# European-XFEL/xFrame

Hardware: AMD Instinct MI355X
Metric: MTIP iterations/sec, 128 q-shells x L_max=32 (higher is better)
Workload: dtype f64 (complex128); 1 GPU; BASELINE config 4: 128 shells x L_max=32, grid 128x64x128, 8 restarts per GPU on 3 streams, tutorial schedule (HIO/SW/ER, ft_stab on), fused step; restarts_per_gpu=8, restarts_total=8, streams_per_gpu=3, engines_take_turns=True, parallelism=restart-sharded x1, step_mode=fused

## Files before the change

### xframe_amd/csrc/k_hankel.hip

```cpp
#include "mtip_internal.h"
#include <vector>

void launch_hankel_mfma(mtip_ctx* c, const double2* in, double2* out, int inverse);

void launch_hankel(mtip_ctx* c, const double2* in, double2* out, int inverse) {
    ProfScope ps(c, "hankel");
    launch_hankel_mfma(c, in, out, inverse);
}

__global__ void __launch_bounds__(256) k_coeff_diff(const double2* __restrict__ a, const double2* __restrict__ b,
                                                    double2* __restrict__ out, int N, int nlm, long long total) {
    const long long idx = (long long)blockIdx.x * blockDim.x + threadIdx.x;
    if (idx >= total) return;
    const int q = (int)((idx / nlm) % N);
    double2 v = a[idx];
    if (q > 0) v = csub(v, b[idx]);
    out[idx] = v;
}

void launch_coeff_diff(mtip_ctx* c, const double2* a, const double2* b, double2* out) {
    const long long total = (long long)c->B * c->N * c->nlm;
    hipLaunchKernelGGL(k_coeff_diff, dim3((unsigned)div_up(total, 256)), dim3(256), 0, c->stream, a, b, out, c->N,
                       c->nlm, total);
}

#define HT_CT_MAX 5
#define HT_KC 16
#define HT_ROWS 128
#define HT_WS (HT_ROWS + 16)
#define HT_THREADS 512
#define HT_NW (HT_KC * HT_ROWS / HT_THREADS)

struct HankelTile32 { int l, cflat0; };

template <int HT_CT, bool SUB>
__global__ void __launch_bounds__(HT_THREADS) k_hankel_tile(const double* __restrict__ in, double* __restrict__ out,
                                                            const double* __restrict__ W,
                                                            const HankelTile32* __restrict__ tiles, int N, int Np, int L,
                                                            int B, int poffs, double scale, int sign,
                                                            const double* __restrict__ in_sub, const uint8_t* __restrict__ sub_mask) {
    constexpr int HT_COLS = 16 * HT_CT;
    constexpr int HT_XS = HT_COLS + 16;
    constexpr int HT_NX = (HT_KC * HT_COLS + HT_THREADS - 1) / HT_THREADS;
    __shared__ double Ws[2][HT_KC][HT_WS];
    __shared__ double Xs[2][HT_KC][HT_XS];
    __shared__ double Ss[SUB ? 2 : 1][SUB ? HT_KC : 1][HT_XS];
    const int tid = threadIdx.x;
    const int wave = tid >> 6, lane = tid & 63;
    const HankelTile32 tinfo = tiles[blockIdx.x];
    const int l = tinfo.l;
    const int k_base = blockIdx.y * HT_ROWS;
    const int ncl = 4 * l + 2;
    const int nlm2 = 2 * (L + 1) * (L + 1);
    const double* Wl = W + (size_t)l * Np * N;
    const int wrow = tid >> 5, wcol = (tid & 31) * 4;
    int xrow[HT_NX], xc[HT_NX];
    size_t xoff[HT_NX];
    bool xok[HT_NX], xsub[HT_NX];
#pragma unroll
    for (int j = 0; j < HT_NX; ++j) {
        const int e = tid + j * HT_THREADS;
        xrow[j] = e / HT_COLS;
        xc[j] = e - xrow[j] * HT_COLS;
        const int cflat = tinfo.cflat0 + xc[j];
        xok[j] = xrow[j] < HT_KC && cflat < B * ncl;
        const int b = xok[j] ? cflat / ncl : 0;
        const int within = xok[j] ? cflat - b * ncl : 0;
        xoff[j] = (size_t)b * N * nlm2 + 2 * (size_t)l * l + within;
        xsub[j] = SUB && (sub_mask == nullptr || sub_mask[b] != 0);
    }
    double rw0[HT_NW], rx0[HT_NX], rw1[HT_NW], rx1[HT_NX];
    double rs0[SUB ? HT_NX : 1], rs1[SUB ? HT_NX : 1];
    auto request = [&](int p0, double (&rw)[HT_NW], double (&rx)[HT_NX], double (&rs)[SUB ? HT_NX : 1]) {
        const int p = p0 + wrow;
        const bool p_ok = p < Np;
        const double* wr = Wl + (size_t)(p_ok ? p : 0) * N + k_base + wcol;
#pragma unroll
        for (int j = 0; j < HT_NW; ++j) rw[j] = (p_ok && k_base + wcol + j < N) ? wr[j] : 0.0;
#pragma unroll
        for (int j = 0; j < HT_NX; ++j) {
            const bool ok = xok[j] && p0 + xrow[j] < Np;
            const size_t o = xoff[j] + (size_t)(p0 + xrow[j] + poffs) * nlm2;
            rx[j] = ok ? in[o] : 0.0;
            if (SUB) {
                rs[j] = (ok && xsub[j]) ? in_sub[o] : 0.0;
                rx[j] -= rs[j];
            }
        }
    };
    auto deposit = [&](int buf, const double (&rw)[HT_NW], const double (&rx)[HT_NX], const double (&rs)[SUB ? HT_NX : 1]) {
#pragma unroll
        for (int j = 0; j < HT_NW; ++j) Ws[buf][wrow][wcol + j] = rw[j];
#pragma unroll
        for (int j = 0; j < HT_NX; ++j)
            if (xrow[j] < HT_KC) {
                Xs[buf][xrow[j]][xc[j]] = rx[j];
                if (SUB) Ss[buf][xrow[j]][xc[j]] = rs[j];
            }
    };
    const int li = lane & 15, kk = lane >> 4;
    v4f64 acc[HT_CT];
#pragma unroll
    for (int t = 0; t < HT_CT; ++t) acc[t] = v4f64{0.0, 0.0, 0.0, 0.0};
    auto multiply = [&](int buf) {
#pragma unroll
        for (int s = 0; s < HT_KC / 4; ++s) {
            const double af = Ws[buf][4 * s + kk][wave * 16 + li];
#pragma unroll
            for (int t = 0; t < HT_CT; ++t) {
                const double bf = Xs[buf][4 * s + kk][16 * t + li];
                acc[t] = __builtin_amdgcn_mfma_f64_16x16x4f64(af, bf, acc[t], 0, 0, 0);
            }
            if (SUB && wave == 0 && k_base == 0) {
                const double a0 = li == 0 ? af : 0.0;
#pragma unroll
                for (int t = 0; t < HT_CT; ++t) {
                    const double sf = Ss[buf][4 * s + kk][16 * t + li];
                    acc[t] = __builtin_amdgcn_mfma_f64_16x16x4f64(a0, sf, acc[t], 0, 0, 0);
                }
            }
        }
    };
    const int n_chunks = (Np + HT_KC - 1) / HT_KC;
    request(0, rw0, rx0, rs0);
    deposit(0, rw0, rx0, rs0);
    if (n_chunks > 1) request(HT_KC, rw1, rx1, rs1);
    if (n_chunks > 2) request(2 * HT_KC, rw0, rx0, rs0);
    __syncthreads();
    for (int i = 0; i < n_chunks; i += 2) {
        multiply(0);
        if (i + 1 < n_chunks) deposit(1, rw1, rx1, rs1);
        __syncthreads();
        if (i + 3 < n_chunks) request((i + 3) * HT_KC, rw1, rx1, rs1);
        if (i + 1 >= n_chunks) break;
        multiply(1);
        if (i + 2 < n_chunks) deposit(0, rw0, rx0, rs0);
        __syncthreads();
        if (i + 4 < n_chunks) request((i + 4) * HT_KC, rw0, rx0, rs0);
    }
    int r = l & 3;
    if (sign < 0) r = (4 - r) & 3;
    const bool is_im = (li & 1) != 0;
#pragma unroll
    for (int t = 0; t < HT_CT; ++t) {
        const int cflat = tinfo.cflat0 + 16 * t + li;
        const bool col_ok = cflat < B * ncl;
        const int b = col_ok ? cflat / ncl : 0;
        const int within = col_ok ? cflat - b * ncl : 0;
        const size_t col_off = (size_t)b * N * nlm2 + 2 * (size_t)l * l + within;
#pragma unroll
        for (int j = 0; j < 4; ++j) {
            double v = acc[t][j] * scale;
            const double partner = __shfl_xor(v, 1, 64);
            double o;
            if (r == 0) o = v;
            else if (r == 2) o = -v;
            else if (r == 1) o = is_im ? partner : -partner;
            else o = is_im ? -partner : partner;
            const int k = k_base + wave * 16 + kk + 4 * j;
            if (col_ok && k < N) out[col_off + (size_t)k * nlm2] = o;
        }
    }
}

bool hankel_has_difference(const mtip_ctx* c) { return c->d_htiles32 != nullptr; }

int hankel_row_blocks(const mtip_ctx* c) { return div_up(c->N, HT_ROWS); }

void launch_hankel_mfma_sub(mtip_ctx* c, const double2* in, const double2* in_sub, double2* out, int inverse, const uint8_t* sub_mask) {
    const dim3 grid((unsigned)c->n_htiles32, (unsigned)hankel_row_blocks(c));
#define HT_LAUNCH(CT, SUBF)                                                                                                  \
    hipLaunchKernelGGL((k_hankel_tile<CT, SUBF>), grid, dim3(HT_THREADS), 0, c->stream, reinterpret_cast<const double*>(in), \
                       reinterpret_cast<double*>(out), (const double*)c->d_W, (const HankelTile32*)c->d_htiles32, c->N,      \
                       c->Np, c->L, c->B, c->cfg.hankel_trapz ? 1 : 0, inverse ? c->inv_scale : c->fwd_scale,                \
                       inverse ? +1 : -1, reinterpret_cast<const double*>(in_sub), sub_mask)
    if (in_sub != nullptr) {
        switch (c->htile_ct) {
            case 1: HT_LAUNCH(1, true); break;
            case 2: HT_LAUNCH(2, true); break;
            case 3: HT_LAUNCH(3, true); break;
            default: HT_LAUNCH(5, true); break;
        }
    } else {
        switch (c->htile_ct) {
            case 1: HT_LAUNCH(1, false); break;
            case 2: HT_LAUNCH(2, false); break;
            case 3: HT_LAUNCH(3, false); break;
            default: HT_LAUNCH(5, false); break;
        }
    }
#undef HT_LAUNCH
}

void launch_hankel_mfma(mtip_ctx* c, const double2* in, double2* out, int inverse) {
    launch_hankel_mfma_sub(c, in, nullptr, out, inverse);
}

int build_hankel_tiles(mtip_ctx* c) {
    std::vector<HankelTile32> t32;
    const int cts[4] = {5, 3, 2, 1};
    for (int ci = 0; ci < 4; ++ci) {
        t32.clear();
        c->htile_ct = cts[ci];
        for (int l = c->L; l >= 0; --l) {
            const int ncols = c->B * (4 * l + 2);
            for (int c0 = 0; c0 < ncols; c0 += 16 * cts[ci]) t32.push_back(HankelTile32{l, c0});
        }
        if (c->htile_force > 0 ? cts[ci] == c->htile_force : (int)t32.size() * hankel_row_blocks(c) * 5 >= c->n_cu * 4) break;
    }
    {
        const int X = 8;
        std::vector<std::vector<HankelTile32>> q(X);
        size_t i0 = 0;
        while (i0 < t32.size()) {
            size_t i1 = i0;
            while (i1 < t32.size() && t32[i1].l == t32[i0].l) ++i1;
            int best = 0;
            for (int x = 1; x < X; ++x)
                if (q[x].size() < q[best].size()) best = x;
            q[best].insert(q[best].end(), t32.begin() + i0, t32.begin() + i1);
            i0 = i1;
        }
        std::vector<size_t> head(X, 0);
        std::vector<HankelTile32> order;
        while (order.size() < t32.size())
            for (int x = 0; x < X && order.size() < t32.size(); ++x) {
                if (head[x] < q[x].size()) { order.push_back(q[x][head[x]++]); continue; }
                int longest = 0;
                for (int y = 1; y < X; ++y)
                    if (q[y].size() - head[y] > q[longest].size() - head[longest]) longest = y;
                order.push_back(q[longest].back());
                q[longest].pop_back();
            }
        t32.swap(order);
    }
    c->n_htiles32 = (int)t32.size();
    if (c->d_htiles32.alloc(t32.size()) != hipSuccess) return MTIP_ENOMEM;
    (void)mtip_copy(c, c->d_htiles32, t32.data(), t32.size() * sizeof(HankelTile32), hipMemcpyHostToDevice);
    return MTIP_OK;
}
```

### xframe_amd/csrc/mtip_api.hip

```cpp
#include "mtip_internal.h"
#include <algorithm>
#include <cmath>
#include <cstdlib>
#include <cstring>

static thread_local std::string g_create_error;

#define CTX_CHECK(c)                       \
    do {                                   \
        if ((c) == nullptr) return MTIP_EINVAL; \
    } while (0)
#define FAIL(c, code, msg)      \
    do {                        \
        (c)->err = (msg);       \
        return (code);          \
    } while (0)

static int post_launch(mtip_ctx* c, const char* what) {
    hipError_t e = hipGetLastError();
    if (e != hipSuccess) {
        c->err = std::string(what) + ": " + hipGetErrorString(e);
        return MTIP_EHIP;
    }
    return MTIP_OK;
}

template <typename T>
static int dev_alloc(mtip_ctx* c, DevBuf<T>* p, size_t n) {
    const hipError_t e = p->alloc(n);
    if (e != hipSuccess) {
        c->err = std::string("hipMalloc: ") + hipGetErrorString(e);
        return MTIP_ENOMEM;
    }
    return MTIP_OK;
}

static ProjSwitches read_proj_switches() {
    ProjSwitches s;
    if (const char* e = std::getenv("MTIP_PROJ_FUSE")) s.fuse = std::atoi(e) != 0;
    if (const char* e = std::getenv("MTIP_JAC_RESIDENT")) s.jac_resident = std::atoi(e) != 0;
    if (const char* e = std::getenv("MTIP_JAC_TG")) s.jac_tg = std::atoi(e) == 8 ? 8 : 16;
    if (const char* e = std::getenv("MTIP_PROJ_REAL")) s.real = std::atoi(e) != 0;
    if (const char* e = std::getenv("MTIP_POLAR_ABS_TOL")) s.polar_abs_tol = std::atof(e);
    if (const char* e = std::getenv("MTIP_RP_CORR")) s.rp_corr = std::atoi(e) != 0;
    if (const char* e = std::getenv("MTIP_RP_EARLY")) s.rp_early = std::min(std::max(std::atof(e), 1e-3), 0.2);
    if (const char* e = std::getenv("MTIP_RP_CORR2_MAX")) s.rp_corr2_max = std::min(std::max(std::atof(e), 1e-6), 5e-4);
    return s;
}

extern "C" {

int mtip_device_count(void) {
    int n = 0;
    if (hipGetDeviceCount(&n) != hipSuccess) return 0;
    return n;
}

const char* mtip_last_error(const mtip_ctx* ctx) { return ctx ? ctx->err.c_str() : g_create_error.c_str(); }

void mtip_destroy(mtip_ctx* c) {
    if (!c) return;
    (void)hipSetDevice(c->device);
    if (c->stream) (void)hipStreamSynchronize(c->stream);
    for (hipEvent_t e : c->prof_events) (void)hipEventDestroy(e);
    if (c->ev0) (void)hipEventDestroy(c->ev0);
    if (c->ev1) (void)hipEventDestroy(c->ev1);
    if (c->turn_ev) (void)hipEventDestroy(c->turn_ev);
    if (c->stream) (void)hipStreamDestroy(c->stream);
    delete c;
}

static int require_loop_band_limit(mtip_ctx* c, const char* what) {
    if (c->L > MTIP_LOOP_L_MAX && !(c->cfg.reserved & MTIP_CFG_LOOP_BIG_L))
        FAIL(c, MTIP_ESTATE, std::string(what) + ": the phasing loop and the projection are built for max_order <= 63; this context has L = " +
                                 std::to_string(c->L) + " and runs the transforms only (DESIGN section 6)");
    return MTIP_OK;
}

static bool is_pow2(int v) { return v > 0 && (v & (v - 1)) == 0; }

mtip_ctx* mtip_create(const mtip_cfg* cfg, int device) {
    if (!cfg) {
        g_create_error = "cfg is NULL";
        return nullptr;
    }
    const int ndev = mtip_device_count();
    if (ndev <= 0) {
        g_create_error = "no HIP device visible (libmtip_hip needs an MI355X; there is no CPU fallback)";
        return nullptr;
    }
    if (device < 0 || device >= ndev) {
        g_create_error = "device index out of range";
        return nullptr;
    }
    if (cfg->n_radial < 2 || cfg->l_max < 0 || cfg->l_max > 128 || cfg->n_batch < 1 || !is_pow2(cfg->n_phi) ||
        cfg->n_phi < 4 || cfg->n_phi > 512 || cfg->n_phi <= 2 * cfg->l_max || cfg->n_theta <= cfg->l_max) {
        g_create_error = "invalid cfg: need Nq>=2, 0<=L<=128 (the transforms; the phasing loop and the projection: L<=63), n_batch>=1, n_phi a power of two in [4,512] and > 2L, n_theta > L";
        return nullptr;
    }
    if (cfg->reserved & ~MTIP_CFG_LOOP_BIG_L) {
        g_create_error = "invalid cfg: reserved is a flag word, only MTIP_CFG_LOOP_BIG_L (bit 0) is defined";
        return nullptr;
    }
    if (hipSetDevice(device) != hipSuccess) {
        g_create_error = "hipSetDevice failed";
        return nullptr;
    }
    mtip_ctx* c = new mtip_ctx();
    c->cfg = *cfg;
    c->device = device;
    c->N = cfg->n_radial;
    c->L = cfg->l_max;
    c->nt = cfg->n_theta;
    c->np = cfg->n_phi;
    c->B = cfg->n_batch;
    c->nlm = (c->L + 1) * (c->L + 1);
    c->nm = 2 * c->L + 1;
    c->Np = cfg->hankel_trapz ? c->N - 1 : c->N;
    c->G = (size_t)c->N * c->nt * c->np;
    c->C = (size_t)c->N * c->nlm;
    const int L = c->L, N = c->N, B = c->B;
    int rc = MTIP_OK;
    auto A = [&](int r) { if (rc == MTIP_OK) rc = r; };
    if (hipStreamCreateWithFlags(&c->stream, hipStreamNonBlocking) != hipSuccess) A(MTIP_EHIP);
    {
        int ncu = 0;
        if (hipDeviceGetAttribute(&ncu, hipDeviceAttributeMultiprocessorCount, device) == hipSuccess && ncu > 0) c->n_cu = ncu;
    }
    (void)hipEventCreate(&c->ev0);
    (void)hipEventCreate(&c->ev1);
    A(dev_alloc(c, &c->d_cost, c->nt));
    A(dev_alloc(c, &c->d_gw, c->nt));
    A(dev_alloc(c, &c->d_P, (size_t)(L + 1) * (L + 2) / 2 * c->nt));
    A(dev_alloc(c, &c->d_poff, L + 2));
    c->npairs = (L + 1) * (L + 2) / 2;
    A(dev_alloc(c, &c->d_PT, (size_t)(c->nt / 2 + 1) * c->npairs));
    A(dev_alloc(c, &c->d_AB, (size_t)c->npairs + L + 1));
    A(dev_alloc(c, &c->d_lmtab, c->npairs));
    A(dev_alloc(c, &c->d_PTc, (size_t)(c->nt / 2 + 1) * 768));
    A(dev_alloc(c, &c->d_lmc, 768));
    if (const char* e = std::getenv("MTIP_DEG2_SIMPLE")) c->deg2_simple = std::atoi(e) != 0;
    if (const char* e = std::getenv("MTIP_HANKEL_CT")) {
        const int v = std::atoi(e);
        c->htile_force = (v == 1 || v == 2 || v == 3 || v == 5) ? v : 0;
    }
    if (rc == MTIP_OK) rc = build_hankel_tiles(c);
    A(dev_alloc(c, &c->d_twN, c->np));
    A(dev_alloc(c, &c->d_tw, c->np / 2));
    A(dev_alloc(c, &c->d_r, N));
    A(dev_alloc(c, &c->d_q, N));
    A(dev_alloc(c, &c->d_W, (size_t)(L + 1) * c->Np * N));
    c->kl.assign(L + 1, 0);
    c->used.assign(L + 1, 0);
    c->active.assign(L + 1, 0);
    c->voff.assign(L + 2, 0);
    c->xoff.assign(L + 2, 0);
    c->uoff.assign(L + 2, 0);
    c->have_V.assign(L + 1, 0);
    c->v_real.assign(L + 1, 1);
    c->psw = read_proj_switches();
    for (int l = 0; l <= L; ++l) {
        const int n = 2 * l + 1, k = std::min(n, N);
        c->kl[l] = k;
        c->voff[l + 1] = c->voff[l] + N * k;
        c->xoff[l + 1] = c->xoff[l] + k * n;
        c->uoff[l + 1] = c->uoff[l] + k * k;
    }
    c->vtot = c->voff[L + 1];
    c->xtot = c->xoff[L + 1];
    c->utot = c->uoff[L + 1];
    A(dev_alloc(c, &c->d_kl, L + 1));
    A(dev_alloc(c, &c->d_used, L + 1));
    A(dev_alloc(c, &c->d_active, L + 1));
    A(dev_alloc(c, &c->d_sweeps, (size_t)B * (L + 1)));
    A(dev_alloc(c, &c->d_voff, L + 2));
    A(dev_alloc(c, &c->d_xoff, L + 2));
    A(dev_alloc(c, &c->d_uoff, L + 2));
    A(dev_alloc(c, &c->d_V, (size_t)c->vtot));
    c->h_V.assign((size_t)c->vtot, make_double2(0.0, 0.0));
    A(dev_alloc(c, &c->d_rmask, (size_t)(L + 1) * N));
    A(dev_alloc(c, &c->d_Bref, (size_t)(L + 1) * N * N));
    A(dev_alloc(c, &c->d_Bnorm, L + 1));
    A(dev_alloc(c, &c->d_deg2_part, (size_t)B * (L + 1) * div_up(N, 16) * div_up(N, 16)));
    A(dev_alloc(c, &c->d_S0, c->G));
    A(dev_alloc(c, &c->d_sup, (size_t)3 * B * c->G));
    A(dev_alloc(c, &c->d_mk, (size_t)3 * B * c->G / 4));
    A(dev_alloc(c, &c->d_err_wr, N));
    A(dev_alloc(c, &c->d_err_wt, c->nt));
    A(dev_alloc(c, &c->d_rho, (size_t)3 * B * c->G));
    A(dev_alloc(c, &c->d_Fp, (size_t)3 * B * c->G));
    A(dev_alloc(c, &c->d_slot, (size_t)B * SL_N));
    A(dev_alloc(c, &c->d_best_err, B));
    A(dev_alloc(c, &c->d_last_err, B));
    A(dev_alloc(c, &c->d_op_err, B));
    A(dev_alloc(c, &c->d_gq, N));
    c->err_cap = 4096;
    A(dev_alloc(c, &c->d_err_hist, (size_t)c->err_cap * B));
    A(dev_alloc(c, &c->d_main_hist, (size_t)c->err_cap * B));
    A(dev_alloc(c, &c->d_deg2_hist, (size_t)c->err_cap * B * (L + 1)));
    A(dev_alloc(c, &c->d_F, (size_t)B * c->G));
    A(dev_alloc(c, &c->d_T1, (size_t)B * c->G));
    A(dev_alloc(c, &c->d_T2, (size_t)B * c->G));
    A(dev_alloc(c, &c->d_fixed, (size_t)B * c->G));
    A(dev_alloc(c, &c->d_g, (size_t)B * N * c->nt * c->nm));
    for (int i = 0; i < 6; ++i) A(dev_alloc(c, &c->d_c[i], (size_t)B * c->C));
    A(dev_alloc(c, &c->d_c0n, (size_t)B * c->C));
    A(dev_alloc(c, &c->d_X, (size_t)B * c->xtot));
    A(dev_alloc(c, &c->d_Vr, (size_t)B * c->utot));
    A(dev_alloc(c, &c->d_U, (size_t)B * c->xtot));
    c->n_partial_blocks = div_up((long long)c->G, 256 * 4);
    A(dev_alloc(c, &c->d_partial, (size_t)B * std::max(c->n_partial_blocks, 2 * N) * 2));
    A(dev_alloc(c, &c->d_minmax, (size_t)B * c->n_partial_blocks * 2));
    if (rc != MTIP_OK) {
        g_create_error = c->err.empty() ? "allocation failed" : c->err;
        mtip_destroy(c);
        return nullptr;
    }
    (void)mtip_copy(c, c->d_kl, c->kl.data(), (L + 1) * sizeof(int), hipMemcpyHostToDevice);
    (void)mtip_copy(c, c->d_voff, c->voff.data(), (L + 2) * sizeof(int), hipMemcpyHostToDevice);
    (void)mtip_copy(c, c->d_xoff, c->xoff.data(), (L + 2) * sizeof(int), hipMemcpyHostToDevice);
    (void)mtip_copy(c, c->d_uoff, c->uoff.data(), (L + 2) * sizeof(int), hipMemcpyHostToDevice);
    (void)hipMemsetAsync(c->d_used, 0, (L + 1) * sizeof(int), c->stream);
    (void)hipMemsetAsync(c->d_active, 0, (L + 1) * sizeof(int), c->stream);
    (void)hipMemsetAsync(c->d_sweeps, 0, (size_t)B * (L + 1) * sizeof(int), c->stream);
    (void)hipMemsetAsync(c->d_U, 0, (size_t)B * c->xtot * sizeof(double2), c->stream);
    (void)hipMemsetAsync(c->d_X, 0, (size_t)B * c->xtot * sizeof(double2), c->stream);
    (void)hipMemsetAsync(c->d_Vr, 0, (size_t)B * c->utot * sizeof(double2), c->stream);
    (void)hipMemsetAsync(c->d_V, 0, (size_t)c->vtot * sizeof(double2), c->stream);
    (void)hipMemsetAsync(c->d_rmask, 0, (size_t)(L + 1) * N, c->stream);
    (void)hipMemsetAsync(c->d_sup, 1, (size_t)3 * B * c->G, c->stream);
    (void)hipMemsetAsync(c->d_S0, 1, c->G, c->stream);
    (void)hipMemsetAsync(c->d_mk, 0xff, (size_t)3 * B * c->G / 4 * sizeof(uint16_t), c->stream);
    std::vector<int> slots((size_t)B * SL_N, 0);
    for (int b = 0; b < B; ++b) {
        slots[b * SL_N + SL_CUR] = 0;
        slots[b * SL_N + SL_OUT] = 1;
        slots[b * SL_N + SL_BEST] = 0;
        slots[b * SL_N + SL_HIST] = 0;
        slots[b * SL_N + SL_ENFORCE] = 1;
    }
    (void)mtip_copy(c, c->d_slot, slots.data(), slots.size() * sizeof(int), hipMemcpyHostToDevice);
    std::vector<double> inf(B, HUGE_VAL);
    (void)mtip_copy(c, c->d_best_err, inf.data(), B * sizeof(double), hipMemcpyHostToDevice);
    (void)mtip_copy(c, c->d_last_err, inf.data(), B * sizeof(double), hipMemcpyHostToDevice);
    return c;
}

int mtip_get_cfg(const mtip_ctx* c, mtip_cfg* out) {
    CTX_CHECK(c);
    if (!out) return MTIP_EINVAL;
    *out = c->cfg;
    return MTIP_OK;
}

int mtip_synchronize(mtip_ctx* c) {
    CTX_CHECK(c);
    MTIP_HIP_CHECK(c, hipStreamSynchronize(c->stream));
    return post_launch(c, "synchronize");
}

int mtip_set_angular_grid(mtip_ctx* c, const double* cos_theta, const double* gauss_weights) {
    CTX_CHECK(c);
    if (!cos_theta || !gauss_weights) FAIL(c, MTIP_EINVAL, "null angular grid");
    (void)hipSetDevice(c->device);
    MTIP_HIP_CHECK(c, mtip_copy(c, c->d_cost, cos_theta, c->nt * sizeof(double), hipMemcpyHostToDevice));
    MTIP_HIP_CHECK(c, mtip_copy(c, c->d_gw, gauss_weights, c->nt * sizeof(double), hipMemcpyHostToDevice));
    build_legendre_tables(c, cos_theta);
    plan_sht(c);
    c->have_angular = true;
    return MTIP_OK;
}

int mtip_set_radial_grid(mtip_ctx* c, const double* r, const double* q) {
    CTX_CHECK(c);
    if (!r || !q) FAIL(c, MTIP_EINVAL, "null radial grid");
    (void)hipSetDevice(c->device);
    MTIP_HIP_CHECK(c, mtip_copy(c, c->d_r, r, c->N * sizeof(double), hipMemcpyHostToDevice));
    MTIP_HIP_CHECK(c, mtip_copy(c, c->d_q, q, c->N * sizeof(double), hipMemcpyHostToDevice));
    c->have_radial = true;
    return MTIP_OK;
}

int mtip_set_hankel_weights(mtip_ctx* c, const double* w_raw, double fwd_scale, double inv_scale) {
    CTX_CHECK(c);
    if (!w_raw) FAIL(c, MTIP_EINVAL, "null weights");
    (void)hipSetDevice(c->device);
    MTIP_HIP_CHECK(c, mtip_copy(c, c->d_W, w_raw, (size_t)(c->L + 1) * c->Np * c->N * sizeof(double), hipMemcpyHostToDevice));
    c->fwd_scale = fwd_scale;
    c->inv_scale = inv_scale;
    c->have_weights = true;
    return MTIP_OK;
}

int mtip_set_projection_matrix(mtip_ctx* c, int l, const mtip_cdouble* V, int k_l, const uint8_t* radial_mask, int used) {
    CTX_CHECK(c);
    if (int r = require_loop_band_limit(c, "mtip_set_projection_matrix")) return r;
    if (l < 0 || l > c->L) FAIL(c, MTIP_EINVAL, "order out of range");
    const int kmax = std::min(2 * l + 1, c->N);
    if (k_l < 1 || k_l > kmax) FAIL(c, MTIP_EINVAL, "k_l must be in [1, min(2l+1, Nq)]");
    if (used && (!V || !radial_mask)) FAIL(c, MTIP_EINVAL, "null projection matrix");
    (void)hipSetDevice(c->device);
    invalidate_projection(c);
    std::vector<double2> tmp((size_t)c->N * kmax, make_double2(0.0, 0.0));
    if (V)
        for (int q = 0; q < c->N; ++q)
            for (int i = 0; i < k_l; ++i) tmp[(size_t)q * kmax + i] = make_double2(V[(size_t)q * k_l + i].re, V[(size_t)q * k_l + i].im);
    double real_tol = 0.0;
    if (const char* e = std::getenv("MTIP_PROJ_REAL_TOL")) real_tol = std::atof(e);
    if (real_tol > 0.0) {
        double vmax = 0.0, imax = 0.0;
        for (const double2& v : tmp) {
            vmax = std::max(vmax, std::max(std::fabs(v.x), std::fabs(v.y)));
            imax = std::max(imax, std::fabs(v.y));
        }
        if (imax <= real_tol * vmax)
            for (double2& v : tmp) v.y = 0.0;
    }
    MTIP_HIP_CHECK(c, mtip_copy(c, c->d_V + c->voff[l], tmp.data(), tmp.size() * sizeof(double2), hipMemcpyHostToDevice));
    std::copy(tmp.begin(), tmp.end(), c->h_V.begin() + c->voff[l]);
    bool is_real = true;
    for (const double2& v : tmp) is_real = is_real && v.y == 0.0;
    c->v_real[l] = is_real ? 1 : 0;
    if (radial_mask) MTIP_HIP_CHECK(c, mtip_copy(c, c->d_rmask + (size_t)l * c->N, radial_mask, c->N, hipMemcpyHostToDevice));
    c->used[l] = used ? 1 : 0;
    bool nonzero = false;
    for (const double2& v : tmp) nonzero = nonzero || v.x != 0.0 || v.y != 0.0;
    c->active[l] = (used && nonzero) ? 1 : 0;
    MTIP_HIP_CHECK(c, mtip_copy(c, c->d_used, c->used.data(), (c->L + 1) * sizeof(int), hipMemcpyHostToDevice));
    MTIP_HIP_CHECK(c, mtip_copy(c, c->d_active, c->active.data(), (c->L + 1) * sizeof(int), hipMemcpyHostToDevice));
    MTIP_HIP_CHECK(c, hipMemsetAsync(c->d_U, 0, (size_t)c->B * c->xtot * sizeof(double2), c->stream));
    c->have_V[l] = 1;
    c->bref_dirty = true;
    return MTIP_OK;
}

int mtip_set_number_of_particles(mtip_ctx* c, double n) {
    CTX_CHECK(c);
    if (!(n > 0)) FAIL(c, MTIP_EINVAL, "number of particles must be > 0");
    c->n_particles = n;
    return MTIP_OK;
}

int mtip_set_so_freedom(mtip_ctx* c, int order) {
    CTX_CHECK(c);
    if (order > c->L || (order >= 0 && (order < 2 || std::min(2 * order + 1, c->N) < 5)))
        FAIL(c, MTIP_EINVAL, "SO_freedom: order must be -1 (off) or an order >= 2 with at least 5 unknown rows");
    c->so_order = order < 0 ? -1 : order;
    return MTIP_OK;
}

static int build_bref(mtip_ctx* c) {
    const int N = c->N, L = c->L;
    std::vector<double2> V((size_t)c->vtot);
    std::vector<uint8_t> rm((size_t)(L + 1) * N);
    MTIP_HIP_CHECK(c, mtip_copy(c, V.data(), c->d_V, V.size() * sizeof(double2), hipMemcpyDeviceToHost));
    MTIP_HIP_CHECK(c, mtip_copy(c, rm.data(), c->d_rmask, rm.size(), hipMemcpyDeviceToHost));
    std::vector<double2> Bref((size_t)(L + 1) * N * N, make_double2(0.0, 0.0));
    std::vector<double> norm(L + 1, 0.0);
    for (int l = 0; l <= L; ++l) {
        const int k = c->kl[l];
        const double2* Vl = V.data() + c->voff[l];
        for (int i = 0; i < N; ++i)
            for (int j = 0; j < N; ++j) {
                if (!(rm[(size_t)l * N + i] && rm[(size_t)l * N + j])) continue;
                double re = 0, im = 0;
                for (int cidx = 0; cidx < k; ++cidx) {
                    const double2 a = Vl[(size_t)i * k + cidx], b = Vl[(size_t)j * k + cidx];
                    re += a.x * b.x + a.y * b.y;
                    im += a.y * b.x - a.x * b.y;
                }
                Bref[((size_t)l * N + i) * N + j] = make_double2(re, im);
                norm[l] += re * re + im * im;
            }
    }
    MTIP_HIP_CHECK(c, mtip_copy(c, c->d_Bref, Bref.data(), Bref.size() * sizeof(double2), hipMemcpyHostToDevice));
    MTIP_HIP_CHECK(c, mtip_copy(c, c->d_Bnorm, norm.data(), norm.size() * sizeof(double), hipMemcpyHostToDevice));
    c->bref_dirty = false;
    return MTIP_OK;
}

int mtip_set_deg2_metric(mtip_ctx* c, int enable) {
    CTX_CHECK(c);
    c->deg2_enable = enable ? 1 : 0;
    return MTIP_OK;
}

int mtip_set_main_error(mtip_ctx* c, int use_reciprocal_deg2, int type) {
    CTX_CHECK(c);
    if (type < 0 || type > 3) FAIL(c, MTIP_EINVAL, "main error type: 0 mean, 1 min, 2 max, 3 prod");
    c->main_mode = use_reciprocal_deg2 ? 1 : 0;
    c->main_type = type;
    return MTIP_OK;
}

int mtip_set_real_constraints(mtip_ctx* c, uint32_t flags, double lo, double hi, double imag_thr, uint32_t hio_flags) {
    CTX_CHECK(c);
    c->rp.flags = flags;
    c->rp.hio_flags = hio_flags;
    c->rp.lo = lo;
    c->rp.hi = hi;
    c->rp.imag_thr = imag_thr;
    return MTIP_OK;
}

int mtip_set_initial_support(mtip_ctx* c, const uint8_t* support) {
    CTX_CHECK(c);
    if (!support) FAIL(c, MTIP_EINVAL, "null support");
    (void)hipSetDevice(c->device);
    MTIP_HIP_CHECK(c, mtip_copy(c, c->d_S0, support, c->G, hipMemcpyHostToDevice));
    std::vector<int> slots((size_t)c->B * SL_N);
    MTIP_HIP_CHECK(c, mtip_copy(c, slots.data(), c->d_slot, slots.size() * sizeof(int), hipMemcpyDeviceToHost));
    for (int b = 0; b < c->B; ++b) {
        slots[b * SL_N + SL_SUP] = 0;
        slots[b * SL_N + SL_SUP_BEST] = 0;
        slots[b * SL_N + SL_ENFORCE] = 1;
        MTIP_HIP_CHECK(c, mtip_copy(c, c->d_sup + (size_t)b * c->G, support, c->G, hipMemcpyHostToDevice));
    }
    MTIP_HIP_CHECK(c, mtip_copy(c, c->d_slot, slots.data(), slots.size() * sizeof(int), hipMemcpyHostToDevice));
    launch_pack_masks(c);
    c->have_support = true;
    return post_launch(c, "mtip_set_initial_support");
}

int mtip_set_error_weights(mtip_ctx* c, const double* radial_w, const double* theta_w, int use_mask) {
    CTX_CHECK(c);
    if (!radial_w || !theta_w) FAIL(c, MTIP_EINVAL, "null error weights");
    (void)hipSetDevice(c->device);
    MTIP_HIP_CHECK(c, mtip_copy(c, c->d_err_wr, radial_w, c->N * sizeof(double), hipMemcpyHostToDevice));
    MTIP_HIP_CHECK(c, mtip_copy(c, c->d_err_wt, theta_w, c->nt * sizeof(double), hipMemcpyHostToDevice));
    c->err_use_mask = use_mask ? 1 : 0;
    c->have_errw = true;
    return MTIP_OK;
}

static int require_transforms(mtip_ctx* c) {
    if (!c->have_angular) FAIL(c, MTIP_ESTATE, "mtip_set_angular_grid has not been called");
    if (!c->have_weights) FAIL(c, MTIP_ESTATE, "mtip_set_hankel_weights has not been called");
    return MTIP_OK;
}
static int require_loop(mtip_ctx* c) {
// ... 882 lines not shown
```

### xframe_amd/csrc/mtip_internal.h

```cpp
#pragma once
#include <hip/hip_runtime.h>
#include <stdint.h>
#include <algorithm>
#include <map>
#include <string>
#include <type_traits>
#include <utility>
#include <vector>
#include "../../include/mtip_hip.h"

#ifndef MTIP_PIN_VGPRS4
#define MTIP_PIN_VGPRS4(a, b, c, d) asm volatile("" : "+v"(a), "+v"(b), "+v"(c), "+v"(d));
#endif
#ifndef MTIP_WAIT_LDS
#define MTIP_WAIT_LDS() asm volatile("s_waitcnt lgkmcnt(0)" ::: "memory")
#endif


#ifndef MTIP_WAVE_LDS_SYNC
#define MTIP_WAVE_LDS_SYNC()                        \
    do {                                            \
        asm volatile("" ::: "memory");              \
        __builtin_amdgcn_wave_barrier();            \
        asm volatile("" ::: "memory");              \
// ... 97 lines not shown
    double2 P = w;
    const bool v_s = f.support & !S;
    P.x = v_s ? 0.0 : P.x;
    P.y = v_s ? 0.0 : P.y;
    const bool c_lo = f.lo & (P.x < rp.lo);
    P.x = c_lo ? rp.lo : P.x;
    const bool c_hi = f.hi & (P.x > rp.hi);
    P.x = c_hi ? rp.hi : P.x;
    const bool v_i = f.imag & (fabs(P.y) >= rp.imag_thr);
    P.y = v_i ? 0.0 : P.y;
    const bool take = f.hio & ((f.h_support & v_s) | (f.h_value & (c_lo | c_hi)) | (f.h_imag & v_i));
    double2 nw;
    nw.x = take ? pv.x - beta * (w.x - P.x) : P.x;
    nw.y = take ? pv.y - beta * (w.y - P.y) : P.y;
    P_out = P;
    return nw;
}

struct RealEpi {
    const double2* prev = nullptr;
    double2* out = nullptr;
    const uint8_t* sup = nullptr;
    const uint8_t* S0 = nullptr;
    const double* wr = nullptr;
    const double* wt = nullptr;
    double* partial = nullptr;
    RealParams rp{};
    int method = 0, err_use_mask = 0, add_prev = 0;
    const uint8_t* add_mask = nullptr;
    double beta = 0.0;
};

enum { EPI_STORE = 0, EPI_MODULUS = 1, EPI_SCALE_SHELL = 2, EPI_MODULUS_FIXED = 3, EPI_REAL_UPDATE = 4 };

struct ProfEntry { double ms = 0; long long n = 0; };

#define MTIP_LOOP_L_MAX 63
#define SHT_BIG_NT_MAX 256
enum { SHT_FWD_GENERIC = 0, SHT_FWD_LDS, SHT_FWD_REG, SHT_FWD_PAIR, SHT_FWD_BIG };
enum { SHT_INV_GENERIC = 0, SHT_INV_LDS, SHT_INV_REG, SHT_INV_WIDE, SHT_INV_BIG };
enum { SHT_CHAIN_OFF = 0, SHT_CHAIN_RT, SHT_CHAIN_REGTAB, SHT_CHAIN_L32 };
struct ShtPlan {
    int fwd = SHT_FWD_GENERIC;
    int fwd_rp = 0;
    int fwd_th = 0;
    int fwd_maxi = 0;
    size_t fwd_lds = 0;
    int inv = SHT_INV_GENERIC;
    int inv_rp = 0;
    int inv_nsplit = 1;
    int inv_jl = 0;
    size_t inv_lds = 0;
    bool real_update = false;
    int real_update_blocks = 0;
    int chain = SHT_CHAIN_OFF;
    int chain_gsz = 0, chain_thg = 0, chain_maxi = 0;
    size_t chain_lds = 0;
};

template <typename T>
struct DevBuf {
    DevBuf() = default;
    DevBuf(DevBuf&& o) noexcept : p_(o.p_) { o.p_ = nullptr; }
    DevBuf& operator=(DevBuf&& o) noexcept {
        if (this != &o) {
            reset();
            swap(o);
        }
        return *this;
    }
    DevBuf(const DevBuf&) = delete;
    DevBuf& operator=(const DevBuf&) = delete;
    ~DevBuf() { reset(); }
    hipError_t alloc(size_t count) {
        reset();
        const hipError_t e = hipMalloc((void**)&p_, std::max<size_t>(count, 1) * sizeof(T));
        if (e != hipSuccess) p_ = nullptr;
        return e;
    }
    void reset() {
        if (p_) (void)hipFree(p_);
        p_ = nullptr;
    }
    void swap(DevBuf& o) noexcept { std::swap(p_, o.p_); }
    operator T*() const { return p_; }

private:
    T* p_ = nullptr;
};
static_assert(!std::is_copy_constructible_v<DevBuf<double>>);

struct JacobiSchedule {
    DevBuf<int> d_tab, d_off, d_rounds;
    int kmax = 0, ps = 0;
    std::vector<int> nrd, off;
};
struct ProjSwitches {
    bool fuse = true;
    bool jac_resident = true;
    int jac_tg = 16;
    bool real = true;
    double polar_abs_tol = 0.0;
    bool rp_corr = true;
    double rp_early = 3e-2, rp_corr2_max = 1.5e-4;
};
struct RpGeom {
    int tg = 16, threads = 256, acc = 0;
    int tab_ints = 0, tab2_entries = 0;
    bool big = false;
    size_t lds = 0;
};

enum { PROJ_JAC_5x16 = 0, PROJ_JAC_9x8, PROJ_JAC_16x8 };
struct ProjPlan {
    bool planned = false, real_ok = false;
    RpGeom rg;
    int kmax = 1, nmax = 1, kmax_used = 1;
    bool fuse = false, lds_path = false, use_sched = false;
    int tg = 16, pad = 0, threads = 64, jac_inst = PROJ_JAC_5x16;
    size_t lds_use = 0, xw_lds = 0, ua_lds = 0;
    DevBuf<int> d_jorder;
    DevBuf<int> d_pg_tiles[6];
    int n_jorder = 0, n_pg_tiles[6] = {0, 0, 0, 0, 0, 0}, rp_n_slots = 0, rp_slot_len = 0;
    DevBuf<double> d_rp_DV, d_rp_Vt;
    DevBuf<int> d_rp_slots;
};
enum { VR_NONE = 0, VR_COMPLEX, VR_REAL };

struct HankelTile32;

struct mtip_ctx {
    mtip_cfg cfg{};
    int device = 0;
    hipStream_t stream = nullptr;
    std::string err;
    int N = 0, L = 0, nt = 0, np = 0, B = 0, nlm = 0, nm = 0, Np = 0;
    size_t G = 0, C = 0;
    DevBuf<double> d_cost, d_gw, d_P, d_r, d_q;
    DevBuf<int> d_poff;
    DevBuf<double2> d_AB;
    DevBuf<double> d_PT;
    DevBuf<double> d_PTc;
    DevBuf<int> d_lmc;
    DevBuf<uint8_t> d_ftmask;
    bool ftmask_mixed = false;
    hipEvent_t turn_ev = nullptr;
    int chain_chunks = 0;
    DevBuf<int> d_lmtab;
    int npairs = 0;
    ShtPlan sht;
    DevBuf<double2> d_twN;
    DevBuf<double2> d_tw;
    DevBuf<double> d_W;
    int n_cu = 256;
    JacobiSchedule js;
    uint32_t im_which = 0;
    DevBuf<uint8_t> d_im_zmask;
    DevBuf<double2> d_im_IIref, d_im_ccdref;
    DevBuf<double> d_rl2_wr, d_rl2_wt, d_rl2_part, d_rl2_hist;
    DevBuf<double> d_im_fq;
    DevBuf<double2> d_im_part;
    DevBuf<double> d_im_qq, d_im_ccdT, d_im_P, d_im_refavg, d_im_refw, d_im_hist;
    double im_ccd_inv_norm = 0.0;
    int so_order = -1;
    DevBuf<long long> d_polar_dbg;
    DevBuf<double2> d_c0n;
    DevBuf<long long> d_chain_dbg;
    bool c0n_valid = false;
    DevBuf<HankelTile32> d_htiles32;
    int htile_force = 0;
    int n_htiles32 = 0, htile_ct = 5;
    double fwd_scale = 0, inv_scale = 0;
    bool have_angular = false, have_radial = false, have_weights = false, have_support = false, have_errw = false;
    ProjSwitches psw;
    ProjPlan pp;
    std::vector<int> kl, used, active, voff, xoff, uoff;
    DevBuf<int> d_active;
    DevBuf<int> d_sweeps;
    std::vector<char> v_real;
    std::vector<double2> h_V;
    int vr = VR_NONE;
    long long proj_calls = 0;
    DevBuf<int> d_kl, d_used, d_voff, d_xoff, d_uoff;
    int vtot = 0, xtot = 0, utot = 0;
    DevBuf<double2> d_V;
    DevBuf<uint8_t> d_rmask;
    std::vector<char> have_V;
    double n_particles = 1.0;
    int deg2_enable = 0;
    DevBuf<double2> d_Bref;
    DevBuf<double> d_Bnorm;
    DevBuf<double> d_deg2_part;
    bool deg2_simple = false;
    bool bref_dirty = true;
    RealParams rp{RC_SUPPORT | RC_VALUE_LO, RC_SUPPORT | RC_VALUE_LO, 0.0, 0.0, 0.0};
    DevBuf<uint8_t> d_S0, d_sup;
    DevBuf<uint16_t> d_mk;
    DevBuf<double> d_err_wr, d_err_wt;
    int err_use_mask = 1;
    DevBuf<double2> d_rho, d_Fp;
    DevBuf<int> d_slot;
    DevBuf<double> d_best_err, d_last_err;
    DevBuf<double> d_op_err;
    DevBuf<double> d_gq;
    DevBuf<double> d_err_hist;
    DevBuf<double> d_main_hist;
    int main_mode = 0, main_type = 0;
    DevBuf<double> d_deg2_hist;
    long long err_cap = 0, n_steps_done = 0;
    bool state_ready = false, fixed_valid = false;
    DevBuf<double2> d_F, d_T1, d_T2;
    DevBuf<double> d_fixed;
    DevBuf<double2> d_g;
    DevBuf<double2> d_c[6];
    DevBuf<double2> d_X, d_Vr, d_U;
    DevBuf<double> d_partial;
    int n_partial_blocks = 0;
    DevBuf<double> d_minmax;
    DevBuf<double2> d_Bl;
    DevBuf<double> d_so3_d;
    DevBuf<double2> d_so3_tw, d_so3_T, d_so3_S, d_so3_P, d_so3_D;
    DevBuf<double> d_so3_C;
    int so3_bw = 0;
    int prof = 0;
    std::map<std::string, ProfEntry> prof_data;
    std::vector<hipEvent_t> prof_events;
    std::vector<std::pair<const char*, int>> prof_pending;
    int prof_next = 0;
    hipEvent_t ev0 = nullptr, ev1 = nullptr;
};

void plan_sht(mtip_ctx* c);
int launch_sht_forward(mtip_ctx* c, const double2* grid, double2* coeff, int prologue, int in_slot = -1);
struct InvEpilogue {
    int mode = EPI_STORE;
    const double2* F = nullptr;
    const double* fixed = nullptr;
    const double* shell_scale = nullptr;
    const double2* coeff_sub = nullptr;
    RealEpi real;
    int out_slot = -1;
};
int launch_sht_inverse(mtip_ctx* c, const double2* coeff, double2* grid, const InvEpilogue& epi);
void build_legendre_tables(mtip_ctx* c, const double* cos_theta);
int sht_no_kernel(mtip_ctx* c, const char* what, int epi_mode);
void launch_sht_forward_fused(mtip_ctx* c, const double2* grid, double2* coeff, int prologue, int in_slot);
int launch_sht_inverse_fused(mtip_ctx* c, const double2* coeff, double2* grid, const InvEpilogue& epi);
void launch_sht_forward_reg(mtip_ctx* c, const double2* grid, double2* coeff, int prologue, int in_slot);
int launch_sht_inverse_reg(mtip_ctx* c, const double2* coeff, double2* grid, const InvEpilogue& epi);
int launch_sht_chain(mtip_ctx* c, const double2* coeff, double2* grid, const InvEpilogue& epi, int prologue, double2* coeff_out);
void launch_hankel(mtip_ctx* c, const double2* in, double2* out, int inverse);
bool hankel_has_difference(const mtip_ctx* c);
void launch_hankel_mfma_sub(mtip_ctx* c, const double2* in, const double2* in_sub, double2* out, int inverse, const uint8_t* sub_mask = nullptr);
int build_jacobi_schedule(mtip_ctx* c, int kmax);
int jacobi_groups(int k);
int build_hankel_tiles(mtip_ctx* c);
int hankel_row_blocks(const mtip_ctx* c);
int launch_invariant_metrics(mtip_ctx* c, const double2* Ilm, long long step);
int launch_reciprocal_l2_metric(mtip_ctx* c, const double2* F, const double2* Fp, long long step);
void launch_deg2(mtip_ctx* c, const double2* Ilm, double2* Bl);
void launch_coeff_diff(mtip_ctx* c, const double2* a, const double2* b, double2* out);
int launch_project_coefficients(mtip_ctx* c, const double2* Ilm, double2* out, bool real_intensity = false);
int require_projection_columns(mtip_ctx* c, const char* what);
void plan_projection(mtip_ctx* c);
void plan_rproj(mtip_ctx* c);
void invalidate_projection(mtip_ctx* c);
int launch_rproj(mtip_ctx* c, double2* coef);
int launch_apply_unknowns(mtip_ctx* c, const double2* Ilm, double2* out);
void launch_deg2_metric(mtip_ctx* c, const double2* Ilm, double* out );
void launch_real_update(mtip_ctx* c, const double2* rho_p, const double2* prev, const double2* rho_rt, double2* out,
                        int method, double beta, int use_slots);
void launch_finish_step(mtip_ctx* c, long long step_index, int nblk = 0);
void launch_abs_to_fixed(mtip_ctx* c);
void launch_modulus_plain(mtip_ctx* c, const double2* F, const double2* Inew, double2* out);
void launch_modulus_fixed_slots(mtip_ctx* c, const double2* F);
void launch_copy_to_slot(mtip_ctx* c, const double2* src, double2* dst_slots, int which);
void launch_sw_clamp(mtip_ctx* c, const double2* conv, double* tmp_real);
void launch_sw_threshold(mtip_ctx* c, const double* tmp_real, double threshold, double error_limit);
void launch_pack_masks(mtip_ctx* c);
void launch_apply_matrix(mtip_ctx* c, const double* M, const double* x, double* y, int nr, int nc, int nv);

#define MTIP_HIP_CHECK(c, call)                                                              \
    do {                                                                                     \
        hipError_t e__ = (call);                                                             \
        if (e__ != hipSuccess) {                                                             \
            (c)->err = std::string(#call) + ": " + hipGetErrorString(e__);                   \
            return MTIP_EHIP;                                                                \
        }                                                                                    \
    } while (0)

void prof_flush(mtip_ctx* c);

struct ProfScope {
    mtip_ctx* c;
    const char* name;
    int idx = -1;
    ProfScope(mtip_ctx* c_, const char* n) : c(c_), name(n) {
        if (!c->prof) return;
        if (c->prof_next + 2 > 8192) prof_flush(c);
        while ((int)c->prof_events.size() < c->prof_next + 2) {
            hipEvent_t e;
            if (hipEventCreateWithFlags(&e, hipEventDisableSystemFence) != hipSuccess) return;
            c->prof_events.push_back(e);
        }
        idx = c->prof_next;
        c->prof_next += 2;
        (void)hipEventRecord(c->prof_events[idx], c->stream);
    }
    ~ProfScope() {
        if (idx < 0) return;
        (void)hipEventRecord(c->prof_events[idx + 1], c->stream);
        c->prof_pending.emplace_back(name, idx);
    }
};

static inline hipError_t mtip_copy(hipStream_t stream, void* dst, const void* src, size_t n) {
    hipError_t e = hipStreamSynchronize(stream);
    if (e != hipSuccess) return e;
    e = hipMemcpy(dst, src, n, hipMemcpyDefault);
    return e != hipSuccess ? e : hipStreamSynchronize(nullptr);
}
static inline hipError_t mtip_copy(mtip_ctx* c, void* dst, const void* src, size_t n, hipMemcpyKind kind) {
    (void)kind;
    return mtip_copy(c->stream, dst, src, n);
}

static inline bool mtip_is_device_pointer(const void* p) {
    hipPointerAttribute_t at;
    const bool is_dev = hipPointerGetAttributes(&at, p) == hipSuccess && at.type == hipMemoryTypeDevice;
    (void)hipGetLastError();
    return is_dev;
}

static inline size_t mtip_free_memory() {
#ifdef __HIPCC__
    size_t fr = 0, tot = 0;
    if (hipMemGetInfo(&fr, &tot) == hipSuccess) return fr;
#endif
    return (size_t)8 << 30;
}

struct DevView {
    mtip_ctx* c = nullptr;
    void* dev = nullptr;
    void* host = nullptr;
    size_t bytes = 0;
    bool writeback = false;
    hipError_t err = hipSuccess;
    DevBuf<char> temp;
    DevView(mtip_ctx* c_, const void* p, size_t n, bool read, bool write) : c(c_), bytes(n), writeback(write) {
        if (p == nullptr || n == 0) return;
        if (mtip_is_device_pointer(p)) {
            dev = const_cast<void*>(p);
            return;
        }
        host = const_cast<void*>(p);
        err = temp.alloc(n);
        dev = temp;
        if (err == hipSuccess && read) err = mtip_copy(c, dev, p, n, hipMemcpyHostToDevice);
    }
    hipError_t finish() {
        if (temp && writeback && err == hipSuccess) err = mtip_copy(c, host, dev, bytes, hipMemcpyDeviceToHost);
        return err;
    }
};

static inline int div_up(long long a, long long b) { return (int)((a + b - 1) / b); }
```

Baseline: 17160 MTIP iterations/s.

## Pre-swizzle Hankel weights into MFMA fragment order and load directly to registers

At weight upload time the Hankel weight matrix is rearranged on the host into a per-wave, per-lane MFMA A-fragment layout. The kernel then loads A operands as double2 straight from global memory into registers, with no shared-memory staging. The X tile is loaded with double2 vector accesses, and the K stage is deepened from 16 to 32/64 rows with a simpler double-buffered loop. This cuts shared-memory traffic and LDS footprint for the weights, at the cost of a second weight copy in device memory and a host-side reorder during setup.

```diff
diff --git a/xframe_amd/csrc/k_hankel.hip b/xframe_amd/csrc/k_hankel.hip
--- a/xframe_amd/csrc/k_hankel.hip
+++ b/xframe_amd/csrc/k_hankel.hip
@@ -25,118 +25,129 @@
 }
 
 #define HT_CT_MAX 5
-#define HT_KC 16
 #define HT_ROWS 128
-#define HT_WS (HT_ROWS + 16)
 #define HT_THREADS 512
-#define HT_NW (HT_KC * HT_ROWS / HT_THREADS)
+#define HT_PPAD 64
 
 struct HankelTile32 { int l, cflat0; };
+
+static inline int hankel_wf_pairs(int Np) { return div_up(Np, HT_PPAD) * (HT_PPAD / 8); }
+
+size_t hankel_wf_doubles(const mtip_ctx* c) {
+    return (size_t)(c->L + 1) * div_up(c->N, HT_ROWS) * (HT_ROWS / 16) * hankel_wf_pairs(c->Np) * 128;
+}
+
+int upload_hankel_fragments(mtip_ctx* c, const double* w_raw) {
+    const int N = c->N, Np = c->Np, nrb = div_up(N, HT_ROWS), nj = hankel_wf_pairs(Np);
+    std::vector<double> wf(hankel_wf_doubles(c), 0.0);
+    size_t o = 0;
+    for (int l = 0; l <= c->L; ++l)
+        for (int rb = 0; rb < nrb; ++rb)
+            for (int w = 0; w < HT_ROWS / 16; ++w)
+                for (int j = 0; j < nj; ++j)
+                    for (int lane = 0; lane < 64; ++lane)
+                        for (int h = 0; h < 2; ++h, ++o) {
+                            const int p = 8 * j + 4 * h + (lane >> 4), k = HT_ROWS * rb + 16 * w + (lane & 15);
+                            if (p < Np && k < N) wf[o] = w_raw[((size_t)l * Np + p) * N + k];
+                        }
+    return mtip_copy(c, c->d_Wf, wf.data(), wf.size() * sizeof(double), hipMemcpyHostToDevice) == hipSuccess ? MTIP_OK : MTIP_EHIP;
+}
 
 template <int HT_CT, bool SUB>
 __global__ void __launch_bounds__(HT_THREADS) k_hankel_tile(const double* __restrict__ in, double* __restrict__ out,
-                                                            const double* __restrict__ W,
+                                                            const double* __restrict__ Wf,
                                                             const HankelTile32* __restrict__ tiles, int N, int Np, int L,
                                                             int B, int poffs, double scale, int sign,
                                                             const double* __restrict__ in_sub, const uint8_t* __restrict__ sub_mask) {
+    constexpr int HT_ST = HT_CT == 1 ? 64 : 32;
     constexpr int HT_COLS = 16 * HT_CT;
-    constexpr int HT_XS = HT_COLS + 16;
-    constexpr int HT_NX = (HT_KC * HT_COLS + HT_THREADS - 1) / HT_THREADS;
-    __shared__ double Ws[2][HT_KC][HT_WS];
-    __shared__ double Xs[2][HT_KC][HT_XS];
-    __shared__ double Ss[SUB ? 2 : 1][SUB ? HT_KC : 1][HT_XS];
+    constexpr int HT_XS = (HT_CT & 1) ? HT_COLS : HT_COLS + 16;
+    constexpr int HT_PW = HT_COLS / 2;
+    constexpr int HT_RP = HT_THREADS / HT_PW;
+    constexpr int HT_NX = (HT_ST + HT_RP - 1) / HT_RP;
+    constexpr int HT_NA = HT_ST / 8;
+    static_assert(HT_PPAD % HT_ST == 0 && HT_ST % 8 == 0 && HT_XS % 32 == 16, "stage and stride rules");
+    __shared__ double Xs[2][HT_ST][HT_XS] __attribute__((aligned(16)));
+    __shared__ double Ss[SUB ? 2 : 1][SUB ? HT_ST : 1][HT_XS] __attribute__((aligned(16)));
     const int tid = threadIdx.x;
-    const int wave = tid >> 6, lane = tid & 63;
+    const int wave = __builtin_amdgcn_readfirstlane(tid >> 6), lane = tid & 63;
     const HankelTile32 tinfo = tiles[blockIdx.x];
     const int l = tinfo.l;
     const int k_base = blockIdx.y * HT_ROWS;
     const int ncl = 4 * l + 2;
     const int nlm2 = 2 * (L + 1) * (L + 1);
-    const double* Wl = W + (size_t)l * Np * N;
-    const int wrow = tid >> 5, wcol = (tid & 31) * 4;
-    int xrow[HT_NX], xc[HT_NX];
-    size_t xoff[HT_NX];
-    bool xok[HT_NX], xsub[HT_NX];
-#pragma unroll
-    for (int j = 0; j < HT_NX; ++j) {
-        const int e = tid + j * HT_THREADS;
-        xrow[j] = e / HT_COLS;
-        xc[j] = e - xrow[j] * HT_COLS;
-        const int cflat = tinfo.cflat0 + xc[j];
-        xok[j] = xrow[j] < HT_KC && cflat < B * ncl;
-        const int b = xok[j] ? cflat / ncl : 0;
-        const int within = xok[j] ? cflat - b * ncl : 0;
-        xoff[j] = (size_t)b * N * nlm2 + 2 * (size_t)l * l + within;
-        xsub[j] = SUB && (sub_mask == nullptr || sub_mask[b] != 0);
-    }
-    double rw0[HT_NW], rx0[HT_NX], rw1[HT_NW], rx1[HT_NX];
-    double rs0[SUB ? HT_NX : 1], rs1[SUB ? HT_NX : 1];
-    auto request = [&](int p0, double (&rw)[HT_NW], double (&rx)[HT_NX], double (&rs)[SUB ? HT_NX : 1]) {
-        const int p = p0 + wrow;
-        const bool p_ok = p < Np;
-        const double* wr = Wl + (size_t)(p_ok ? p : 0) * N + k_base + wcol;
-#pragma unroll
-        for (int j = 0; j < HT_NW; ++j) rw[j] = (p_ok && k_base + wcol + j < N) ? wr[j] : 0.0;
-#pragma unroll
-        for (int j = 0; j < HT_NX; ++j) {
-            const bool ok = xok[j] && p0 + xrow[j] < Np;
-            const size_t o = xoff[j] + (size_t)(p0 + xrow[j] + poffs) * nlm2;
-            rx[j] = ok ? in[o] : 0.0;
-            if (SUB) {
-                rs[j] = (ok && xsub[j]) ? in_sub[o] : 0.0;
-                rx[j] -= rs[j];
-            }
-        }
-    };
-    auto deposit = [&](int buf, const double (&rw)[HT_NW], const double (&rx)[HT_NX], const double (&rs)[SUB ? HT_NX : 1]) {
-#pragma unroll
-        for (int j = 0; j < HT_NW; ++j) Ws[buf][wrow][wcol + j] = rw[j];
-#pragma unroll
-        for (int j = 0; j < HT_NX; ++j)
-            if (xrow[j] < HT_KC) {
-                Xs[buf][xrow[j]][xc[j]] = rx[j];
-                if (SUB) Ss[buf][xrow[j]][xc[j]] = rs[j];
-            }
-    };
+    const double2* Wa = reinterpret_cast<const double2*>(Wf) +
+                        (((size_t)l * gridDim.y + blockIdx.y) * (HT_ROWS / 16) + wave) * ((Np + HT_PPAD - 1) / HT_PPAD * (HT_PPAD / 8)) * 64 + lane;
+    const int prow = tid / HT_PW, pc = tid - prow * HT_PW;
+    const int cflat_x = tinfo.cflat0 + 2 * pc;
+    const bool xok = prow < HT_RP && cflat_x < B * ncl;
+    const int xb = xok ? cflat_x / ncl : 0;
+    const size_t xoff = (size_t)xb * N * nlm2 + 2 * (size_t)l * l + (xok ? cflat_x - xb * ncl : 0);
+    const bool xsub = SUB && (sub_mask == nullptr || sub_mask[xb] != 0);
     const int li = lane & 15, kk = lane >> 4;
     v4f64 acc[HT_CT];
 #pragma unroll
     for (int t = 0; t < HT_CT; ++t) acc[t] = v4f64{0.0, 0.0, 0.0, 0.0};
-    auto multiply = [&](int buf) {
-#pragma unroll
-        for (int s = 0; s < HT_KC / 4; ++s) {
-            const double af = Ws[buf][4 * s + kk][wave * 16 + li];
+    double2 a0[HT_NA], a1[HT_NA], rx0[HT_NX], rx1[HT_NX], rs0[SUB ? HT_NX : 1], rs1[SUB ? HT_NX : 1];
+    auto request = [&](int p0, double2 (&a)[HT_NA], double2 (&rx)[HT_NX], double2 (&rs)[SUB ? HT_NX : 1]) {
+        const double2* wa = Wa + (size_t)(p0 / 8) * 64;
+#pragma unroll
+        for (int j = 0; j < HT_NA; ++j) a[j] = wa[(size_t)j * 64];
+#pragma unroll
+        for (int j = 0; j < HT_NX; ++j) {
+            const int row = prow + j * HT_RP;
+            const bool ok = xok && ((j + 1) * HT_RP <= HT_ST || row < HT_ST) && p0 + row < Np;
+            const size_t o = xoff + (size_t)(p0 + row + poffs) * nlm2;
+            rx[j] = ok ? *reinterpret_cast<const double2*>(in + o) : make_double2(0.0, 0.0);
+            if (SUB) rs[j] = (ok && xsub) ? *reinterpret_cast<const double2*>(in_sub + o) : make_double2(0.0, 0.0);
+        }
+    };
+    auto deposit = [&](int buf, const double2 (&rx)[HT_NX], const double2 (&rs)[SUB ? HT_NX : 1]) {
+#pragma unroll
+        for (int j = 0; j < HT_NX; ++j) {
+            const int row = prow + j * HT_RP;
+            if ((HT_RP * HT_PW == HT_THREADS || prow < HT_RP) && ((j + 1) * HT_RP <= HT_ST || row < HT_ST)) {
+                double2 d = rx[j];
+                if (SUB) {
+                    d.x -= rs[j].x;
+                    d.y -= rs[j].y;
+                    *reinterpret_cast<double2*>(&Ss[buf][row][2 * pc]) = rs[j];
+                }
+                *reinterpret_cast<double2*>(&Xs[buf][row][2 * pc]) = d;
+            }
+        }
+    };
+    auto multiply = [&](int buf, const double2 (&a)[HT_NA]) {
+#pragma unroll
+        for (int s = 0; s < HT_ST / 4; ++s) {
+            const double af = (s & 1) ? a[s >> 1].y : a[s >> 1].x;
 #pragma unroll
             for (int t = 0; t < HT_CT; ++t) {
                 const double bf = Xs[buf][4 * s + kk][16 * t + li];
                 acc[t] = __builtin_amdgcn_mfma_f64_16x16x4f64(af, bf, acc[t], 0, 0, 0);
             }
             if (SUB && wave == 0 && k_base == 0) {
-                const double a0 = li == 0 ? af : 0.0;
+                const double a0m = li == 0 ? af : 0.0;
 #pragma unroll
                 for (int t = 0; t < HT_CT; ++t) {
                     const double sf = Ss[buf][4 * s + kk][16 * t + li];
-                    acc[t] = __builtin_amdgcn_mfma_f64_16x16x4f64(a0, sf, acc[t], 0, 0, 0);
+                    acc[t] = __builtin_amdgcn_mfma_f64_16x16x4f64(a0m, sf, acc[t], 0, 0, 0);
                 }
             }
         }
     };
-    const int n_chunks = (Np + HT_KC - 1) / HT_KC;
-    request(0, rw0, rx0, rs0);
-    deposit(0, rw0, rx0, rs0);
-    if (n_chunks > 1) request(HT_KC, rw1, rx1, rs1);
-    if (n_chunks > 2) request(2 * HT_KC, rw0, rx0, rs0);
-    __syncthreads();
-    for (int i = 0; i < n_chunks; i += 2) {
-        multiply(0);
-        if (i + 1 < n_chunks) deposit(1, rw1, rx1, rs1);
+    request(0, a0, rx0, rs0);
+#pragma unroll 1
+    for (int p0 = 0; p0 < Np; p0 += 2 * HT_ST) {
+        deposit(0, rx0, rs0);
+        if (p0 + HT_ST < Np) request(p0 + HT_ST, a1, rx1, rs1);
         __syncthreads();
-        if (i + 3 < n_chunks) request((i + 3) * HT_KC, rw1, rx1, rs1);
-        if (i + 1 >= n_chunks) break;
-        multiply(1);
-        if (i + 2 < n_chunks) deposit(0, rw0, rx0, rs0);
+        multiply(0, a0);
+        if (p0 + HT_ST >= Np) break;
+        deposit(1, rx1, rs1);
+        if (p0 + 2 * HT_ST < Np) request(p0 + 2 * HT_ST, a0, rx0, rs0);
         __syncthreads();
-        if (i + 4 < n_chunks) request((i + 4) * HT_KC, rw0, rx0, rs0);
+        multiply(1, a1);
     }
     int r = l & 3;
     if (sign < 0) r = (4 - r) & 3;
@@ -171,7 +182,7 @@
     const dim3 grid((unsigned)c->n_htiles32, (unsigned)hankel_row_blocks(c));
 #define HT_LAUNCH(CT, SUBF)                                                                                                  \
     hipLaunchKernelGGL((k_hankel_tile<CT, SUBF>), grid, dim3(HT_THREADS), 0, c->stream, reinterpret_cast<const double*>(in), \
-                       reinterpret_cast<double*>(out), (const double*)c->d_W, (const HankelTile32*)c->d_htiles32, c->N,      \
+                       reinterpret_cast<double*>(out), (const double*)c->d_Wf, (const HankelTile32*)c->d_htiles32, c->N,      \
                        c->Np, c->L, c->B, c->cfg.hankel_trapz ? 1 : 0, inverse ? c->inv_scale : c->fwd_scale,                \
                        inverse ? +1 : -1, reinterpret_cast<const double*>(in_sub), sub_mask)
     if (in_sub != nullptr) {
diff --git a/xframe_amd/csrc/mtip_api.hip b/xframe_amd/csrc/mtip_api.hip
--- a/xframe_amd/csrc/mtip_api.hip
+++ b/xframe_amd/csrc/mtip_api.hip
@@ -150,6 +150,7 @@
     A(dev_alloc(c, &c->d_r, N));
     A(dev_alloc(c, &c->d_q, N));
     A(dev_alloc(c, &c->d_W, (size_t)(L + 1) * c->Np * N));
+    A(dev_alloc(c, &c->d_Wf, hankel_wf_doubles(c)));
     c->kl.assign(L + 1, 0);
     c->used.assign(L + 1, 0);
     c->active.assign(L + 1, 0);
@@ -286,6 +287,7 @@
     if (!w_raw) FAIL(c, MTIP_EINVAL, "null weights");
     (void)hipSetDevice(c->device);
     MTIP_HIP_CHECK(c, mtip_copy(c, c->d_W, w_raw, (size_t)(c->L + 1) * c->Np * c->N * sizeof(double), hipMemcpyHostToDevice));
+    if (upload_hankel_fragments(c, w_raw) != MTIP_OK) FAIL(c, MTIP_EHIP, "upload of the fragment-ordered Hankel weights failed");
     c->fwd_scale = fwd_scale;
     c->inv_scale = inv_scale;
     c->have_weights = true;
diff --git a/xframe_amd/csrc/mtip_internal.h b/xframe_amd/csrc/mtip_internal.h
--- a/xframe_amd/csrc/mtip_internal.h
+++ b/xframe_amd/csrc/mtip_internal.h
@@ -273,6 +273,7 @@
     DevBuf<double2> d_twN;
     DevBuf<double2> d_tw;
     DevBuf<double> d_W;
+    DevBuf<double> d_Wf;
     int n_cu = 256;
     JacobiSchedule js;
     uint32_t im_which = 0;
@@ -376,6 +377,8 @@
 int build_jacobi_schedule(mtip_ctx* c, int kmax);
 int jacobi_groups(int k);
 int build_hankel_tiles(mtip_ctx* c);
+size_t hankel_wf_doubles(const mtip_ctx* c);
+int upload_hankel_fragments(mtip_ctx* c, const double* w_raw);
 int hankel_row_blocks(const mtip_ctx* c);
 int launch_invariant_metrics(mtip_ctx* c, const double2* Ilm, long long step);
 int launch_reciprocal_l2_metric(mtip_ctx* c, const double2* F, const double2* Fp, long long step);
```

Measured after the change: 17690 MTIP iterations/s, median of 6. +3.1%, better.
